# UBC-AWP/vision-sam3-yolo-lameless

Measured on AMD Instinct MI355X. Metric: frames/sec (whole node) for YOLO+SAM3+DINOv3 feature extraction, 1080p clips, higher is better.
Workload: dtype f16; 1 GPU; BASELINE cfg#5, dense schedule: fused per-frame path on a synthetic 5 s @ 30 fps 1080p clip (150 unique BGR frames resident in HBM): YOLOv8-l detect (letterbox 384x640, NMS, scale_boxes; f16 plan) -> SAM (Hiera-B+ image encoder + FPN at 1024x1024, box-prompted mask decoder, 1080p mask + statistics + contour features) + DINOv3 ViT-L/16 embed (224x224) on EVERY frame; per-frame records packed, gathe; parallelism=one clip per GPU, 1 GPU(s), one gather per step, streams=7

## Files before the change

### include/lmx.h

```cpp
#ifndef LMX_H
#define LMX_H
#include <stdint.h>
#ifdef __cplusplus
extern "C" {
#endif

#define LMX_VERSION 100

#define LMX_OK 0
#define LMX_EINVAL (-1)
#define LMX_EHIP (-2)

typedef void* lmx_stream_t;

int lmx_version(void);
const char* lmx_last_error(void);
int lmx_device_count(void);

enum { LMX_F16 = 0, LMX_F32 = 1 };
enum { LMX_ACT_NONE = 0, LMX_ACT_SILU = 1, LMX_ACT_GELU = 2 , LMX_ACT_RELU = 3,
       LMX_ACT_SWIGLU = 4  };

typedef struct {
  const void* A;
// ... 76 lines not shown
int lmx_k_nms(const float* pred, int n, int A, int nc, float conf, double iou, int max_det, float max_wh,
              float* boxes, float* scores, int32_t* cls, int32_t* src, int32_t* counts, void* workspace,
              lmx_stream_t stream);

int lmx_k_letterbox(const uint8_t* src, uint8_t* dst, int n, int sh, int sw, int rh, int rw, int top, int left,
                    int oh, int ow, const int32_t* xofs, const int16_t* ialpha, const int32_t* yofs,
                    const int16_t* ibeta, int swap_rb, lmx_stream_t stream);
int lmx_k_stem_conv(const uint8_t* img, const float* w, const float* bias, void* out, int n, int H, int W, int Cout,
                    lmx_stream_t stream);
int lmx_k_maxpool5(const void* src, int64_t lds, void* dst, int64_t ldd, int n, int H, int W, int C,
                   lmx_stream_t stream);
int lmx_k_upsample2(const void* src, int64_t lds, void* dst, int64_t ldd, int n, int H, int W, int C,
                    lmx_stream_t stream);
int lmx_k_detect_decode(const float* head, int64_t ldh, float* pred, int n, int H, int W, int nc, float stride,
                        int a_off, int A, lmx_stream_t stream);
int lmx_k_scale_boxes(float* boxes, int total, float padx, float pady, float gain, float w, float h,
                      lmx_stream_t stream);

int lmx_k_split3(const float* x, int64_t ldx, int act, const void* res3, int64_t ldr, void* out3, int64_t ldo, int64_t rows,
                 int N, int g, int nsum, int64_t sum_stride, lmx_stream_t stream);
int lmx_k_maxpool5_x3(const void* src3, int64_t lds, void* dst3, int64_t ldd, int n, int H, int W, int C, lmx_stream_t stream);
int lmx_k_stem_conv_x3(const uint8_t* img, const float* w, const float* bias, void* out3, int n, int H, int W, int Cout,
                       lmx_stream_t stream);
int lmx_k_attention_f32(const float* q, int64_t ldq, const float* k, int64_t ldk, const float* v, int64_t ldv, float* o,
                        int64_t ldo, int B, int H, int Tq, int Tk, int hd, float scale, lmx_stream_t stream);
int lmx_k_hyper_mask_f32(const float* up, const float* hyper, float* logits, int n, int G, int C, int act, lmx_stream_t stream);

int lmx_k_pose_gather(const float* raw0, const float* raw1, const float* raw2, int64_t ldk, const int32_t* hw,
                      const float* strides, const int32_t* src, const int32_t* counts, int n, int max_det, int K, int ndim,
                      float padx, float pady, float gain, float w, float h, float* out, lmx_stream_t stream);

int lmx_k_im2col_u8(const uint8_t* img, const float* lut, void* out, int n, int rh, int rw, int IH, int IW, int KH,
                    int KW, int stride, int pad, int64_t ldo, lmx_stream_t stream);
int lmx_k_maxpool2(const void* src, int64_t lds, void* dst, int64_t ldd, int dtype, int n, int H, int W, int C,
                   lmx_stream_t stream);
int lmx_k_cast_f32_f16(const float* src, int64_t lds, void* dst, int64_t ldd, int64_t rows, int cols,
                       lmx_stream_t stream);

int lmx_k_add_bcast(const void* a, int a_dtype, int64_t lda, const float* b, int64_t ldb, int b_rows, void* out,
                    int out_dtype, int64_t ldo, int64_t rows, int D, lmx_stream_t stream);
int lmx_k_prompt_box(const float* boxes, int64_t ldb, float* sparse, int n, double sx, double sy, float S,
                     const float* gauss, const float* corner, int F, lmx_stream_t stream);
int lmx_k_hyper_mask(const void* up, const float* hyper, float* logits, int n, int G, int C, lmx_stream_t stream);
int lmx_k_mask_post(const float* logits, int n, int L, int T, int nh, int nw, int h, int w, uint8_t* mask,
                    int64_t* stats, float* workspace, lmx_stream_t stream);
int lmx_k_prompt_points(const float* points, const int32_t* labels, int Np, const float* boxes, int64_t ldb, float* sparse, int n,
                        double sx, double sy, float S, const float* gauss, const float* point_embed, const float* not_a_point,
                        const float* corner, int F, lmx_stream_t stream);
#define LMX_MASK_EMBED_PARAMS 4684
int lmx_k_mask_embed(const float* mask_input, const void* emb, int emb_dtype, int64_t lde, const float* params, float* keys,
                     int64_t ldk, int n, int G, lmx_stream_t stream);
int lmx_k_hyper_mask_multi(const void* up, const float* hyper, float* logits, int n, int M, int G, int C, lmx_stream_t stream);
int lmx_k_hyper_mask_multi_f32(const float* up, const float* hyper, float* logits, int n, int M, int G, int C, int act,
                               lmx_stream_t stream);
int lmx_k_mask_logits(const float* logits, int n, int L, int T, int nh, int nw, int h, int w, float* out, lmx_stream_t stream);

int lmx_k_mask_score(const float* logits, int n, int L, int T, int nh, int nw, int h, int w, double thr, double off,
                     const int32_t* idx, int64_t* out, lmx_stream_t stream);
int lmx_k_nms_boxes(const float* boxes, int64_t ldb, const float* scores, const uint8_t* valid, int n, double iou, int32_t* keep_out,
                    int32_t* count_out, void* workspace, lmx_stream_t stream);
int lmx_k_pack_bits(const uint8_t* src, int64_t rows, int w, uint8_t* dst, lmx_stream_t stream);

int64_t lmx_contour_workspace_bytes(int n, int h, int w);
int lmx_k_contour_features(const uint8_t* mask, int n, int h, int w, int64_t* out, void* workspace, lmx_stream_t stream);

int lmx_h_mask_features(const uint8_t* mask_host, int h, int w, double* out_host);
// ... 9 lines not shown
```

### vision-sam3-yolo-lameless_amd/csrc/nms.hip

```cpp
#include "common.h"

namespace {

constexpr int MAX_A = 16384;

__global__ __launch_bounds__(256) void nms_filter_kernel(const float* __restrict__ pred, int n, int A, int nc,
                                                         float conf, unsigned long long* __restrict__ keys,
                                                         int* __restrict__ counts) {
  const int64_t total = (int64_t)n * A;
  const int row_len = 4 + nc;
  for (int64_t i = (int64_t)blockIdx.x * blockDim.x + threadIdx.x; i < total; i += (int64_t)gridDim.x * blockDim.x) {
    const int img = (int)(i / A);
    const int a = (int)(i - (int64_t)img * A);
    const float* row = pred + i * row_len + 4;
    float best = row[0];
    for (int c = 1; c < nc; ++c) {
      const float v = row[c];
      best = v > best ? v : best;
    }
    if (best > conf) {
      const int slot = atomicAdd(&counts[img], 1);
      const unsigned long long key =
          ((unsigned long long)__float_as_uint(best) << 32) | (unsigned long long)(0xFFFFFFFFu - (unsigned)a);
      keys[(int64_t)img * A + slot] = key;
    }
  }
}

struct Box {
  float x1, y1, x2, y2, area;
};

__device__ __forceinline__ bool iou_gt(const Box& a, const Box& b, double thr) {
  const float xx1 = a.x1 > b.x1 ? a.x1 : b.x1;
  const float yy1 = a.y1 > b.y1 ? a.y1 : b.y1;
  const float xx2 = a.x2 < b.x2 ? a.x2 : b.x2;
  const float yy2 = a.y2 < b.y2 ? a.y2 : b.y2;
  float w = xx2 - xx1;
  w = w > 0.f ? w : 0.f;
  float h = yy2 - yy1;
  h = h > 0.f ? h : 0.f;
  const float inter = w * h;
  const float ovr = inter / (a.area + b.area - inter);
  return (double)ovr > thr;
}

__device__ __forceinline__ void bitonic_sort_desc(unsigned long long* keys, int npow2) {
  const int tid = threadIdx.x;
  for (int k = 2; k <= npow2; k <<= 1) {
    for (int j = k >> 1; j > 0; j >>= 1) {
      for (int i = tid; i < npow2; i += 1024) {
        const int ixj = i ^ j;
        if (ixj > i) {
          const unsigned long long a = keys[i], b = keys[ixj];
          const bool desc = (i & k) == 0;
          if (desc ? (a < b) : (a > b)) {
            keys[i] = b;
// ... 199 lines not shown
    sbox[i * 5 + 2] = r[2];
    sbox[i * 5 + 3] = r[3];
    sbox[i * 5 + 4] = (r[2] - r[0]) * (r[3] - r[1]);
  }
  __syncthreads();

  const int total = greedy_blocks(sbox, count, iou, count, supp, kept, [&](int, int i, int o) {
    keep_out[o] = (int)(0xFFFFFFFFu - (unsigned)(keys[i] & 0xFFFFFFFFull));
  });
  if (tid == 0) count_out[0] = total;
}

}

extern "C" int64_t lmx_nms_workspace_bytes(int n, int A) {
  if (n <= 0 || A <= 0) return 0;
  return 256 + ((int64_t)n * 4 + 255) / 256 * 256 + (int64_t)n * A * 8 + (int64_t)n * A * 5 * 4;
}

extern "C" int lmx_k_nms(const float* pred, int n, int A, int nc, float conf, double iou, int max_det, float max_wh,
                         float* boxes, float* scores, int32_t* cls, int32_t* src, int32_t* counts, void* workspace,
                         lmx_stream_t stream) {
  LMX_REQUIRE(pred && boxes && scores && cls && src && counts && workspace, "lmx_k_nms: null pointer");
  LMX_REQUIRE(n > 0 && A > 0 && A <= MAX_A && nc > 0 && max_det > 0, "lmx_k_nms: n=%d A=%d (<=%d) nc=%d max_det=%d", n,
              A, MAX_A, nc, max_det);
  LMX_REQUIRE((((uintptr_t)workspace) & 255) == 0, "lmx_k_nms: workspace must be 256-byte aligned");
  hipStream_t st = reinterpret_cast<hipStream_t>(stream);
  char* ws = reinterpret_cast<char*>(workspace);
  int* cand_counts = reinterpret_cast<int*>(ws);
  const int64_t cnt_bytes = ((int64_t)n * 4 + 255) / 256 * 256;
  unsigned long long* keys = reinterpret_cast<unsigned long long*>(ws + cnt_bytes);
  float* sbox = reinterpret_cast<float*>(ws + cnt_bytes + (int64_t)n * A * 8);
  LMX_HIP(hipMemsetAsync(cand_counts, 0, (size_t)n * 4, st));
  int64_t g = ((int64_t)n * A + 255) / 256;
  if (g > 2048) g = 2048;
  hipLaunchKernelGGL(nms_filter_kernel, dim3((unsigned)g), dim3(256), 0, st, pred, n, A, nc, conf, keys, cand_counts);
  int rc = lmx_launch_check("nms_filter_kernel");
  if (rc) return rc;
  int npow2 = 64;
  while (npow2 < A) npow2 <<= 1;
  const size_t smem = (size_t)npow2 * 9 + 64 * sizeof(Box);
  int dev;
  LMX_TRY(lmx_stream_device(st, &dev));
  LMX_TRY(lmx_allow_lds(reinterpret_cast<const void*>(&nms_greedy_kernel), (int)((size_t)MAX_A * 9 + 64 * sizeof(Box)), dev));
  hipLaunchKernelGGL(nms_greedy_kernel, dim3(n), dim3(1024), smem, st, pred, A, nc, iou, max_det, max_wh, keys, cand_counts,
                     sbox, boxes, scores, cls, src, counts);
  return lmx_launch_check("nms_greedy_kernel");
}

extern "C" int lmx_k_nms_boxes(const float* boxes, int64_t ldb, const float* scores, const uint8_t* valid, int n, double iou,
                               int32_t* keep_out, int32_t* count_out, void* workspace, lmx_stream_t stream) {
  LMX_REQUIRE(boxes && scores && keep_out && count_out && workspace, "lmx_k_nms_boxes: null pointer");
  LMX_REQUIRE(n > 0 && n <= MAX_A && ldb >= 4, "lmx_k_nms_boxes: n=%d (1..%d) ldb=%lld", n, MAX_A, (long long)ldb);
  LMX_REQUIRE((((uintptr_t)workspace) & 15) == 0, "lmx_k_nms_boxes: workspace must be 16-byte aligned");
  int npow2 = 64;
  while (npow2 < n) npow2 <<= 1;
  const size_t smem = (size_t)npow2 * 9 + 64 * sizeof(Box);
  hipStream_t st = reinterpret_cast<hipStream_t>(stream);
  int dev;
  LMX_TRY(lmx_stream_device(st, &dev));
  LMX_TRY(lmx_allow_lds(reinterpret_cast<const void*>(&nms_boxes_kernel), (int)((size_t)MAX_A * 9 + 64 * sizeof(Box)), dev));
  hipLaunchKernelGGL(nms_boxes_kernel, dim3(1), dim3(1024), smem, st, boxes, ldb, scores, valid, n, iou, reinterpret_cast<float*>(workspace),
                     keep_out, count_out);
  return lmx_launch_check("nms_boxes_kernel");
}
```

### vision-sam3-yolo-lameless_amd/csrc/sam.hip

```cpp
#include "common.h"

namespace {

inline int grid_for(int64_t total, int block = 256) {
  int64_t g = (total + block - 1) / block;
  if (g > 256 * 8) g = 256 * 8;
  if (g < 1) g = 1;
  return (int)g;
}

template <int KW_T>
__global__ __launch_bounds__(256) void im2col_u8_kernel(const uint8_t* __restrict__ img, const float* __restrict__ lut,
                                                        half_t* __restrict__ out, int n, int rh, int rw, int OH, int OW, int KH,
                                                        int KW_rt, int stride, int pad, int64_t ldo) {
  __shared__ float lut_s[768];
  for (int i = threadIdx.x; i < 768; i += blockDim.x) lut_s[i] = lut[i];
  __syncthreads();
  const int KW = KW_T > 0 ? KW_T : KW_rt;
  const int chunks = (int)(ldo / 8);
  const int K = KH * KW * 3;
  const int64_t total = (int64_t)n * OH * OW * chunks;
  for (int64_t i = (int64_t)blockIdx.x * blockDim.x + threadIdx.x; i < total; i += (int64_t)gridDim.x * blockDim.x) {
    const int ck = (int)(i % chunks);
    const int64_t tok = i / chunks;
// ... 253 lines not shown
    if (fast) {
      x = *reinterpret_cast<const unsigned long long*>(sp);
    } else {
      for (int e = 0; e < 8; ++e)
        if (c * 8 + e < w) x |= (unsigned long long)sp[e] << (8 * e);
    }
    x = (x | (x >> 1) | (x >> 2) | (x >> 3) | (x >> 4) | (x >> 5) | (x >> 6) | (x >> 7)) & 0x0101010101010101ull;
    dst[i] = (uint8_t)((x * 0x8040201008040201ull) >> 56);
  }
}

__global__ __launch_bounds__(256) void prompt_box_kernel(const float* __restrict__ boxes, int64_t ldb, float* __restrict__ sparse,
                                                        int n, double sx, double sy, float S, const float* __restrict__ gauss,
                                                        const float* __restrict__ corner, int F) {
  const int i = blockIdx.x * blockDim.x + threadIdx.x;
  if (i >= n * 2 * F) return;
  const int j = i % F, k = (i / F) & 1, b = i / (2 * F);
  const float* bx = boxes + (int64_t)b * ldb + 2 * k;
  const float px = (float)((double)bx[0] * sx) + 0.5f, py = (float)((double)bx[1] * sy) + 0.5f;
  const float cx = 2.f * (px / S) - 1.f, cy = 2.f * (py / S) - 1.f;
  const float ang = 6.283185307179586f * (cx * gauss[j] + cy * gauss[F + j]);
  float* o = sparse + ((int64_t)b * 2 + k) * 2 * F;
  o[j] = sinf(ang) + corner[k * 2 * F + j];
  o[F + j] = cosf(ang) + corner[k * 2 * F + F + j];
}

__global__ void mask_stats_init_kernel(long long* stats, int n) {
  const int i = blockIdx.x * blockDim.x + threadIdx.x;
  if (i >= n * 8) return;
  const int f = i & 7;
  stats[i] = (f == 3 || f == 4) ? 0x7fffffffll : ((f == 5 || f == 6) ? -1ll : 0ll);
}

}

extern "C" int lmx_k_im2col_u8(const uint8_t* img, const float* lut, void* out, int n, int rh, int rw, int IH, int IW, int KH,
                               int KW, int stride, int pad, int64_t ldo, lmx_stream_t stream) {
  LMX_REQUIRE(img && lut && out, "lmx_k_im2col_u8: null pointer");
  LMX_REQUIRE(n > 0 && rh > 0 && rw > 0 && rh <= IH && rw <= IW && KH > 0 && KW > 0 && stride > 0 && pad >= 0,
              "lmx_k_im2col_u8: geometry");
  LMX_REQUIRE(ldo % 8 == 0 && ldo >= (int64_t)KH * KW * 3 && aligned16(out), "lmx_k_im2col_u8: ldo/alignment");
  const int OH = (IH + 2 * pad - KH) / stride + 1, OW = (IW + 2 * pad - KW) / stride + 1;
  LMX_REQUIRE((int64_t)rh * rw * 3 < 0x7fffffffll, "lmx_k_im2col_u8: frame too large");
  const dim3 grid(grid_for((int64_t)n * OH * OW * (ldo / 8)));
  hipStream_t st = reinterpret_cast<hipStream_t>(stream);
  half_t* o16 = reinterpret_cast<half_t*>(out);
  if (KW == 7)
    hipLaunchKernelGGL((im2col_u8_kernel<7>), grid, dim3(256), 0, st, img, lut, o16, n, rh, rw, OH, OW, KH, KW, stride, pad, ldo);
  else if (KW == 16)
    hipLaunchKernelGGL((im2col_u8_kernel<16>), grid, dim3(256), 0, st, img, lut, o16, n, rh, rw, OH, OW, KH, KW, stride, pad, ldo);
  else
    hipLaunchKernelGGL((im2col_u8_kernel<0>), grid, dim3(256), 0, st, img, lut, o16, n, rh, rw, OH, OW, KH, KW, stride, pad, ldo);
  return lmx_launch_check("im2col_u8_kernel");
}

extern "C" int lmx_k_maxpool2(const void* src, int64_t lds, void* dst, int64_t ldd, int dtype, int n, int H, int W, int C,
                              lmx_stream_t stream) {
  LMX_REQUIRE(src && dst, "lmx_k_maxpool2: null pointer");
  LMX_REQUIRE(n > 0 && H > 0 && W > 0 && H % 2 == 0 && W % 2 == 0 && C > 0 && lds >= C && ldd >= C, "lmx_k_maxpool2: shape");
  hipStream_t st = reinterpret_cast<hipStream_t>(stream);
  if (dtype == LMX_F16) {
    LMX_REQUIRE(C % 8 == 0 && lds % 8 == 0 && ldd % 8 == 0 && aligned16(src) && aligned16(dst), "lmx_k_maxpool2: f16 alignment");
    hipLaunchKernelGGL((maxpool2_kernel<half_t, 8>), dim3(grid_for((int64_t)n * (H / 2) * (W / 2) * (C / 8))), dim3(256), 0, st,
                       reinterpret_cast<const half_t*>(src), lds, reinterpret_cast<half_t*>(dst), ldd, n, H, W, C);
  } else if (dtype == LMX_F32) {
    LMX_REQUIRE(C % 4 == 0 && lds % 4 == 0 && ldd % 4 == 0 && aligned16(src) && aligned16(dst), "lmx_k_maxpool2: f32 alignment");
    hipLaunchKernelGGL((maxpool2_kernel<float, 4>), dim3(grid_for((int64_t)n * (H / 2) * (W / 2) * (C / 4))), dim3(256), 0, st,
                       reinterpret_cast<const float*>(src), lds, reinterpret_cast<float*>(dst), ldd, n, H, W, C);
  } else {
    LMX_REQUIRE(false, "lmx_k_maxpool2: dtype %d", dtype);
  }
  return lmx_launch_check("maxpool2_kernel");
}

extern "C" int lmx_k_cast_f32_f16(const float* src, int64_t lds, void* dst, int64_t ldd, int64_t rows, int cols,
                                  lmx_stream_t stream) {
  LMX_REQUIRE(src && dst, "lmx_k_cast_f32_f16: null pointer");
  LMX_REQUIRE(rows > 0 && cols > 0 && cols % 4 == 0 && lds % 4 == 0 && ldd % 4 == 0 && lds >= cols && ldd >= cols,
              "lmx_k_cast_f32_f16: shape");
  LMX_REQUIRE(aligned16(src) && ((((uintptr_t)dst) & 7) == 0), "lmx_k_cast_f32_f16: alignment");
  hipLaunchKernelGGL(cast_kernel, dim3(grid_for(rows * (cols / 4))), dim3(256), 0, reinterpret_cast<hipStream_t>(stream), src, lds,
                     reinterpret_cast<half_t*>(dst), ldd, rows, cols);
  return lmx_launch_check("cast_kernel");
}

extern "C" int lmx_k_prompt_box(const float* boxes, int64_t ldb, float* sparse, int n, double sx, double sy, float S,
// ... 81 lines not shown
```

### vision-sam3-yolo-lameless_amd/lmx/_lib.py

```python
import ctypes as C
import os

_HERE = os.path.dirname(os.path.abspath(__file__))
LIB_PATH = os.environ.get("LMX_LIB") or os.path.join(_HERE, "liblmx.so")


class LmxError(RuntimeError):
    pass


class GemmDesc(C.Structure):
    _fields_ = [
        ("A", C.c_void_p), ("W", C.c_void_p), ("bias", C.c_void_p), ("scale", C.c_void_p), ("res", C.c_void_p),
        ("C", C.c_void_p),
        ("lda", C.c_int64), ("ldc", C.c_int64), ("ldr", C.c_int64),
        ("M", C.c_int32), ("N", C.c_int32), ("K", C.c_int32),
        ("act", C.c_int32), ("out_dtype", C.c_int32), ("a_mode", C.c_int32),
        ("H", C.c_int32), ("W_", C.c_int32), ("Cin", C.c_int32), ("conv_stride", C.c_int32),
        ("Ho", C.c_int32), ("Wo", C.c_int32), ("res_rows", C.c_int32), ("a_rep", C.c_int32), ("split_k", C.c_int32), ("split_stride", C.c_int64),
    ]


class AttnDesc(C.Structure):
    _fields_ = [
# ... 16 lines not shown
    "lmx_dbg_set_gemm2_variant": (None, [_I]),
    "lmx_k_pose_gather": (_I, [_VP, _VP, _VP, _I64, _VP, _VP, _VP, _VP, _I, _I, _I, _I, _F, _F, _F, _F, _F, _VP, _VP]),
    "lmx_k_pack_bits": (_I, [_VP, _I64, _I, _VP, _VP]),
    "lmx_k_ln_mlp": (_I, [_VP, _I64, _VP, _VP, _VP, _VP, _VP, _VP, _I64, _I, _F, _VP, _VP, _VP, _VP, _VP, _VP]),
    "lmx_k_hiera_attn8": (_I, [_VP, _VP, _I64, _VP, _VP, _F, _VP, _VP, _VP, _VP, _I, _I, _I, _I, _I, _F, _VP]),
    "lmx_k_hiera_attn4": (_I, [_VP, _VP, _I64, _VP, _VP, _I, _I, _I, _I, _I, _F, _VP]),
    "lmx_k_hiera_attn_pool": (_I, [_VP, _VP, _VP, _VP, _I, _I, _I, _I, _I, _I, _F, _VP]),
    "lmx_k_ln_mlp_img": (_I, [_VP, _I64, _VP, _VP, _I64, _I, _F, _VP, _VP, _VP]),
    "lmx_k_layernorm": (_I, [_VP, _I, _I64, _VP, _VP, _VP, _I, _I64, _I, _I, _F, _I, _VP]),
    "lmx_k_attention": (_I, [C.POINTER(AttnDesc), _VP]),
    "lmx_k_relpos_tables": (_I, [C.POINTER(AttnDesc), _VP, _VP, _I, _VP, _VP]),
    "lmx_k_rope": (_I, [_VP, _I64, _I, _I, _I, _I, _I, _VP, _VP, _VP]),
    "lmx_k_pil_resize_h": (_I, [_VP, _VP, _I, _I, _I, _I, _VP, _VP, _I, _I, _VP]),
    "lmx_k_pil_resize_v": (_I, [_VP, _VP, _I, _I, _I, _I, _VP, _VP, _I, _VP]),
    "lmx_k_patchify_norm": (_I, [_VP, _VP, _I, _I, _I, _I, _I, _I, _I, _I, _I64, _VP, _VP]),
    "lmx_k_float_resize_patchify": (_I, [_VP, _VP, _I, _I, _I, _I, _I, _I, _I64, _VP, _VP, _I, _VP, _VP, _I, _I, _F, _VP, _I, _VP]),
    "lmx_k_assemble_tokens": (_I, [_VP, _VP, _VP, _VP, _I, _I, _I, _I, _VP]),
    "lmx_k_token_mean": (_I, [_VP, _I, _VP, _I, _I, _I, _VP]),
    "lmx_k_swiglu": (_I, [_VP, _I64, _VP, _I64, _I, _I, _VP]),
    "lmx_nms_workspace_bytes": (_I64, [_I, _I]),
    "lmx_k_nms": (_I, [_VP, _I, _I, _I, _F, _D, _I, _F, _VP, _VP, _VP, _VP, _VP, _VP, _VP]),
    "lmx_k_letterbox": (_I, [_VP, _VP, _I, _I, _I, _I, _I, _I, _I, _I, _I, _VP, _VP, _VP, _VP, _I, _VP]),
    "lmx_k_stem_conv": (_I, [_VP, _VP, _VP, _VP, _I, _I, _I, _I, _VP]),
    "lmx_k_split3": (_I, [_VP, _I64, _I, _VP, _I64, _VP, _I64, _I64, _I, _I, _I, _I64, _VP]),
    "lmx_k_maxpool5_x3": (_I, [_VP, _I64, _VP, _I64, _I, _I, _I, _I, _VP]),
    "lmx_k_stem_conv_x3": (_I, [_VP, _VP, _VP, _VP, _I, _I, _I, _I, _VP]),
    "lmx_k_attention_f32": (_I, [_VP, _I64, _VP, _I64, _VP, _I64, _VP, _I64, _I, _I, _I, _I, _I, _F, _VP]),
    "lmx_k_hyper_mask_f32": (_I, [_VP, _VP, _VP, _I, _I, _I, _I, _VP]),
    "lmx_k_maxpool5": (_I, [_VP, _I64, _VP, _I64, _I, _I, _I, _I, _VP]),
    "lmx_k_upsample2": (_I, [_VP, _I64, _VP, _I64, _I, _I, _I, _I, _VP]),
    "lmx_k_detect_decode": (_I, [_VP, _I64, _VP, _I, _I, _I, _I, _F, _I, _I, _VP]),
    "lmx_k_scale_boxes": (_I, [_VP, _I, _F, _F, _F, _F, _F, _VP]),
    "lmx_k_im2col_u8": (_I, [_VP, _VP, _VP, _I, _I, _I, _I, _I, _I, _I, _I, _I, _I64, _VP]),
    "lmx_k_maxpool2": (_I, [_VP, _I64, _VP, _I64, _I, _I, _I, _I, _I, _VP]),
    "lmx_k_cast_f32_f16": (_I, [_VP, _I64, _VP, _I64, _I64, _I, _VP]),
    "lmx_k_add_bcast": (_I, [_VP, _I, _I64, _VP, _I64, _I, _VP, _I, _I64, _I64, _I, _VP]),
    "lmx_h_mask_features": (_I, [_VP, _I, _I, _VP]),
    "lmx_h_iou_matrix": (_I, [_VP, _I, _VP, _I, _VP]),
    "lmx_h_assign": (_I, [_VP, _I, _I, _VP, _VP]),
    "lmx_contour_workspace_bytes": (_I64, [_I, _I, _I]),
    "lmx_k_contour_features": (_I, [_VP, _I, _I, _I, _VP, _VP, _VP]),
    "lmx_k_prompt_box": (_I, [_VP, _I64, _VP, _I, _D, _D, _F, _VP, _VP, _I, _VP]),
    "lmx_k_hyper_mask": (_I, [_VP, _VP, _VP, _I, _I, _I, _VP]),
    "lmx_k_mask_post": (_I, [_VP, _I, _I, _I, _I, _I, _I, _I, _VP, _VP, _VP, _VP]),
    "lmx_k_prompt_points": (_I, [_VP, _VP, _I, _VP, _I64, _VP, _I, _D, _D, _F, _VP, _VP, _VP, _VP, _I, _VP]),
    "lmx_k_mask_embed": (_I, [_VP, _VP, _I, _I64, _VP, _VP, _I64, _I, _I, _VP]),
    "lmx_k_hyper_mask_multi": (_I, [_VP, _VP, _VP, _I, _I, _I, _I, _VP]),
    "lmx_k_hyper_mask_multi_f32": (_I, [_VP, _VP, _VP, _I, _I, _I, _I, _I, _VP]),
    "lmx_k_mask_logits": (_I, [_VP, _I, _I, _I, _I, _I, _I, _I, _VP, _VP]),
    "lmx_k_mask_score": (_I, [_VP, _I, _I, _I, _I, _I, _I, _I, _D, _D, _VP, _VP, _VP]),
    "lmx_k_nms_boxes": (_I, [_VP, _I64, _VP, _VP, _I, _D, _VP, _VP, _VP, _VP]),
}

_lib = None


def load():
    global _lib
    if _lib is not None:
        return _lib
    if not os.path.exists(LIB_PATH):
        raise ImportError(
            f"{LIB_PATH} not found: build it with `python -c 'import __graft_entry__ as g; g.build()'` "
            "(hipcc --offload-arch=gfx950).  lmx has no CPU fallback.")
    import torch

# ... 14 lines not shown
```

### vision-sam3-yolo-lameless_amd/lmx/kernels.py

```python
import ctypes as C
import os
import threading

import torch

from . import _lib
from ._lib import AttnDesc, GemmDesc, LmxError, check

F16, F32 = 0, 1
ACT_NONE, ACT_SILU, ACT_GELU, ACT_RELU, ACT_SWIGLU = 0, 1, 2, 3, 4
_DT = {torch.float16: F16, torch.float32: F32}


_tls = threading.local()


def _stream(dev):
    _tls.dev = dev
    return C.c_void_p(torch.cuda.current_stream(dev).cuda_stream)


def _ptr(t):
    return C.c_void_p(t.data_ptr()) if t is not None else C.c_void_p(0)

# ... 42 lines not shown
        raise LmxError(f"gemm: out shape {tuple(out.shape)} != ({Mout},{Nout})")
    d = GemmDesc()
    d.A, d.W, d.C = a.data_ptr(), w.data_ptr(), out.data_ptr()
    d.bias = bias.data_ptr() if bias is not None else None
    d.scale = scale.data_ptr() if scale is not None else None
    d.lda, d.ldc, d.ldr = lda, ldc, 0
    if bias is not None and (bias.dtype != torch.float32 or bias.numel() != N):
        raise LmxError("gemm: bias must be float32 [N]")
    if scale is not None and (scale.dtype != torch.float32 or scale.numel() != Nout):
        raise LmxError("gemm: scale must be float32 [N] (ACT_SWIGLU: [N/2])")
    if res is not None:
        Mr, Nr, ldr = _rows(res, "gemm res")
        if (Mr, Nr) != ((res_rows or M), N) or res.dtype != out.dtype:
            raise LmxError("gemm: residual must match out's shape and dtype")
        d.res, d.ldr = res.data_ptr(), ldr
    d.res_rows = res_rows
    d.M, d.N, d.K = M, N, a_rep * K
    d.act, d.out_dtype, d.a_mode, d.a_rep = act, _DT[out.dtype], 0, a_rep
    if pool_hw:
        d.a_mode, d.H, d.W_ = 2, int(pool_hw[0]), int(pool_hw[1])
    check(_lib.load().lmx_k_gemm(C.byref(d), _stream(dev)), "lmx_k_gemm")
    return out


def im2col_u8(img, lut, IH, IW, KH, KW, stride, pad, ldo):
    dev = _dev(img, lut)
    n, rh, rw, c = img.shape
    if c != 3 or img.dtype != torch.uint8 or not img.is_contiguous():
        raise LmxError("im2col_u8: img must be contiguous uint8 [n,h,w,3]")
    OH, OW = (IH + 2 * pad - KH) // stride + 1, (IW + 2 * pad - KW) // stride + 1
    out = torch.empty((n * OH * OW, ldo), dtype=torch.float16, device=img.device)
    check(_lib.load().lmx_k_im2col_u8(_ptr(img), _ptr(lut), _ptr(out), n, rh, rw, IH, IW, KH, KW, stride, pad, ldo,
                                      _stream(dev)), "lmx_k_im2col_u8")
    return out


def maxpool2(x, out):
    dev = _dev(x, out)
    n, H, W, Cc, ps = _nhwc(x, "maxpool2 x")
    no, Ho, Wo, Co, pso = _nhwc(out, "maxpool2 out")
    if (no, Ho, Wo, Co) != (n, H // 2, W // 2, Cc) or x.dtype != out.dtype:
        raise LmxError("maxpool2: shape/dtype mismatch")
    check(_lib.load().lmx_k_maxpool2(_ptr(x), ps, _ptr(out), pso, _DT[x.dtype], n, H, W, Cc, _stream(dev)), "lmx_k_maxpool2")
    return out


def cast_f16(x, out=None):
    dev = _dev(x, out)
    rows, cols, lds = _rows(x, "cast src")
    if out is None:
        out = torch.empty((rows, cols), dtype=torch.float16, device=x.device)
    check(_lib.load().lmx_k_cast_f32_f16(_ptr(x), lds, _ptr(out), out.stride(0), rows, cols, _stream(dev)),
          "lmx_k_cast_f32_f16")
    return out


def _nhwc(t, what):
    if t.dim() != 4 or t.stride(3) != 1:
        raise LmxError(f"{what}: expected NHWC with contiguous channels, got {tuple(t.shape)} / {t.stride()}")
    n, H, W, Cc = t.shape
    ps = t.stride(2)
    if t.stride(1) != W * ps or (n > 1 and t.stride(0) != H * W * ps):
        raise LmxError(f"{what}: not a channel slice of a dense NHWC buffer: strides {t.stride()}")
    return n, H, W, Cc, ps


# ... 661 lines not shown
                                      _stream(dev)), "lmx_k_nms_boxes")
    return keep, count


def contour_features(mask):
    dev = _dev(mask)
    if mask.dtype != torch.uint8 or mask.dim() != 3 or not mask.is_contiguous():
        raise LmxError("contour_features: mask must be contiguous uint8 [n,h,w]")
    n, h, w = mask.shape
    lib = _lib.load()
    ws = torch.empty((int(lib.lmx_contour_workspace_bytes(n, h, w)),), dtype=torch.uint8, device=mask.device)
    out = torch.empty((n, 8), dtype=torch.int64, device=mask.device)
    check(lib.lmx_k_contour_features(_ptr(mask), n, h, w, _ptr(out), _ptr(ws), _stream(dev)), "lmx_k_contour_features")
    return out


LAUNCH_TRACE = None
_raw_lib = None
RIDGE_FLOP_PER_BYTE = 2500e12 / 8e12


def _work(name, args):
    if name == "lmx_k_gemm":
        d = args[0]._obj
        M, N, Kd = d.M, d.N, d.K
        osz = 4 if d.out_dtype == F32 else 2
        a_bytes = 2 * M * (Kd // max(d.a_rep, 1))
        if d.a_mode == 1:
            a_bytes = 2 * (M // max(d.Ho * d.Wo, 1)) * d.H * d.W_ * d.Cin
        by = a_bytes + 2 * N * Kd + osz * (M // 4 if d.a_mode == 2 else M) * (N // 2 if d.act == ACT_SWIGLU else N) + (osz * (d.res_rows or M) * N if d.res else 0)
        fl = 2.0 * M * N * Kd
        key = f"gemm M={M} N={N} K={Kd} out={'f32' if osz == 4 else 'f16'} conv3x3={d.a_mode} act={d.act} res={int(bool(d.res))}"
        return ("gemm/mfma-bound" if fl / by >= RIDGE_FLOP_PER_BYTE else "gemm/hbm-bound"), fl, by, key
    if name == "lmx_k_attention":
        d = args[0]._obj
        fl = 4.0 * d.B * d.H * d.Tq * d.Tk * d.hd
        by = 2 * d.H * d.hd * d.B * (2 * d.Tq + 2 * d.Tk)
        key = f"attention B={d.B} H={d.H} Tq={d.Tq} Tk={d.Tk} hd={d.hd} mode={d.mode} ws={d.ws} qs={d.q_stride} rel={int(bool(d.rel))}"
        return ("attention/mfma-bound" if fl / by >= RIDGE_FLOP_PER_BYTE else "attention/hbm-bound"), fl, by, key
    if name == "lmx_k_layernorm":
        in_dt, out_dt, rows, D = args[1], args[6], args[8], args[9]
        return "layernorm", 0.0, rows * D * ((4 if in_dt == F32 else 2) + (4 if out_dt == F32 else 2)), f"layernorm rows={rows} D={D} in={in_dt} out={out_dt}"
    if name == "lmx_k_ln_mlp_img":
        rows, D = args[4], args[5]
        return "fused ln+mlp", 16.0 * D * D * rows, (8 + (2 if args[7] else 0) + (2 if args[8] else 0)) * D * rows, f"ln_mlp_img rows={rows} D={D}"
    if name == "lmx_k_ln_mlp":
        rows, D = args[8], args[9]
        return "fused ln+mlp", 16.0 * D * D * rows, (16 + (2 if args[12] else 0) + (2 if args[15] else 0)) * D * rows, f"ln_mlp rows={rows} D={D}"
    if name == "lmx_k_hiera_attn8":
        n_, Gh, Gw, D = args[10], args[11], args[12], args[13]
        rows = n_ * Gh * Gw
        return "fused attention half", rows * (8.0 * D * D + 256.0 * D), rows * D * (8 + (2 if args[0] else 0)), f"hiera_attn8 rows={rows} D={D} ln_inside={int(not args[0])}"
    if name == "lmx_k_hiera_attn4":
        n_, Gh, Gw, D = args[5], args[6], args[7], args[8]
        rows = n_ * Gh * Gw
        return "fused attention half", rows * (8.0 * D * D + 64.0 * D), rows * D * 10, f"hiera_attn4 rows={rows} D={D}"
    if name == "lmx_k_hiera_attn_pool":
        n_, Gh, Gw, Di, Do = args[4], args[5], args[6], args[7], args[8]
        rows = n_ * Gh * Gw
        keys = 64 if Di == 112 else 16
        return "fused attention half", rows * (8.0 * Di * Do + keys * Do + 0.5 * Do * Do), rows * (2 * Di + Do), f"hiera_attn_pool rows={rows} {Di}->{Do}"
    if name == "lmx_k_cast_f32_f16":
        rows, cols = args[4], args[5]
        return "streaming glue", 0.0, 6 * rows * cols, f"cast_f32_f16 rows={rows} cols={cols}"
    if name == "lmx_k_maxpool2":
        dt, n_, H, W, C_ = args[4], args[5], args[6], args[7], args[8]
# ... 67 lines not shown
```

### vision-sam3-yolo-lameless_amd/lmx/sam.py

```python
import math
import os
from dataclasses import dataclass

import numpy as np
import torch

from . import kernels as K
from . import resample

SAM_PIXEL_MEAN = (123.675, 116.28, 103.53)
SAM_PIXEL_STD = (58.395, 57.12, 57.375)


@dataclass
class HieraConfig:
    hidden: int = 112
    blocks: tuple = (2, 3, 16, 3)
    dims: tuple = (112, 224, 448, 896)
    heads: tuple = (2, 4, 8, 16)
    windows: tuple = (8, 4, 14, 7)
    global_blocks: tuple = (12, 16, 20)
    pos_bkg: tuple = (14, 14)
    q_pool_stages: int = 3
    fpn_dim: int = 256
# ... 267 lines not shown
                nx = f"backbone.blocks.{i + 1}." if i + 1 < len(self.blocks) else None
                f32 = lambda k: np.asarray(sd[k], np.float32)
                blk["mlp_img"] = tuple(torch.from_numpy(a).to(dev) for a in pack_ln_mlp(
                    f32(p + "mlp.proj_in.weight"), f32(p + "mlp.proj_in.bias"), f32(p + "mlp.proj_out.weight"), f32(p + "mlp.proj_out.bias"),
                    f32(p + "layer_norm2.weight"), f32(p + "layer_norm2.bias"),
                    f32(nx + "layer_norm1.weight") if nx else None, f32(nx + "layer_norm1.bias") if nx else None))
        n = len(cfg.dims) - 1
        self.neck = [(t16(sd[f"neck.convs.{n - i}.weight"][:, :, 0, 0]), t32(sd[f"neck.convs.{n - i}.bias"])) for i in range(n + 1)]
        self.lut = t32(sam_norm_lut())
        self._tabs = {}

    def _tables(self, h, w):
        key = (h, w)
        if key not in self._tabs:
            nh, nw = resize_longest_side(h, w, self.cfg.image)
            dev = self.device

            def up(tab):
                b, k, ks = tab
                return (torch.from_numpy(b).to(dev), torch.from_numpy(k).to(dev), ks)

            th = up(resample.coeff_tables(w, nw, resample.BILINEAR)) if nw != w else None
            tv = up(resample.coeff_tables(h, nh, resample.BILINEAR)) if nh != h else None
            self._tabs[key] = (nh, nw, th, tv)
        return self._tabs[key]

    def preprocess(self, frames):
        n, h, w, _ = frames.shape
        nh, nw, th, tv = self._tables(h, w)
        img = K.pil_resize(frames, nw, nh, th, tv, swap_rb=False)
        S = self.cfg.image
        return img, K.im2col_u8(img, self.lut, S, S, 7, 7, 4, 3, self.k_pad)

    def trunk(self, patches, n):
        cfg = self.cfg
        g = self.grid0
        x = K.gemm(patches, self.pe_w, bias=self.pe_b, res=self.pos, res_rows=g * g, out_dtype=torch.float32)
        H = W = g
        stage_ends = set(int(v) for v in np.cumsum(cfg.blocks) - 1)
        stages, stages16 = [], []
        dev = x.device
        h_next = None
        for i, B in enumerate(self.blocks):
            dim, D, heads, qs = B["dim"], B["dim_out"], B["heads"], B["qs"]
            rows = n * H * W
            if self._attn8(i, H, W):
                if B["attn8_ln"]:
                    K.hiera_attn8(x, B["attn8"], n, H, W, heads, ln=(B["g1"], B["b1"], cfg.eps))
                else:
                    K.hiera_attn8(x, B["attn8"], n, H, W, heads, h=h_next if h_next is not None else K.layernorm(x, B["g1"], B["b1"], cfg.eps))
            elif "attnp" in B and K.hiera_attn_pool_ok(dim, D, heads, B["win"], H, W, qs):
                x = K.hiera_attn_pool(h_next if h_next is not None else K.layernorm(x, B["g1"], B["b1"], cfg.eps), B["attnp"], n, H, W, heads, D)
                H, W = H // 2, W // 2
            elif "attn4" in B and K.hiera_attn4_ok(D, heads, B["win"], H, W, qs):
                K.hiera_attn4(h_next if h_next is not None else K.layernorm(x, B["g1"], B["b1"], cfg.eps), x, B["attn4"], n, H, W, heads)
            else:
                h = h_next if h_next is not None else K.layernorm(x, B["g1"], B["b1"], cfg.eps)
                if dim != D:
                    if qs and K.pooled_gemm_ok(rows, D):
                        sc = K.gemm(h, B["wp"], bias=B["bp"], out_dtype=torch.float32, pool_hw=(H, W))
                    else:
                        sc = K.gemm(h, B["wp"], bias=B["bp"], out_dtype=torch.float32)
                        if qs:
                            pooled = torch.empty((n, H // 2, W // 2, D), dtype=torch.float32, device=dev)
                            K.maxpool2(sc.view(n, H, W, D), pooled)
                            sc = pooled.view(-1, D)
                    res = sc
                else:
                    res = x
                x, H, W = self._attention_half(B, h, x, res, n, H, W)
# ... 52 lines not shown
                        window=dict(Gh=H, Gw=W, ws=win, q_stride=2 if qs else 1),
                        pad_k=B["padkv"][D:2 * D], pad_v=B["padkv"][2 * D:])
        else:
            K.attention(q, k, v, a, n, heads, Hq * Wq, H * W, hd, hd ** -0.5)
        xo = torch.empty((n * Hq * Wq, D), dtype=torch.float32, device=dev) if res is not x else x
        K.gemm(a, B["wo"], bias=B["bo"], res=res, out=xo)
        return xo, Hq, Wq

    def fpn(self, stages, stages16=None):
        cfg = self.cfg
        nlev = len(stages) - 1
        feats, prev = [], None
        for i in range(nlev, -1, -1):
            s = stages[i]
            n, H, W, C = s.shape
            a = stages16[i] if stages16 and stages16[i] is not None else K.cast_f16(s.view(-1, C))
            w, b = self.neck[i]
            out = torch.empty((n, H, W, cfg.fpn_dim), dtype=torch.float16, device=s.device)
            if i not in cfg.fpn_top_down or i == nlev:
                K.gemm(a, w, bias=b, out=out.view(-1, cfg.fpn_dim))
            else:
                up = torch.empty((n, H, W, cfg.fpn_dim), dtype=torch.float16, device=s.device)
                K.upsample2(prev, up)
                K.gemm(a, w, bias=b, res=up.view(-1, cfg.fpn_dim), out=out.view(-1, cfg.fpn_dim))
            prev = out
            feats.append(out)
        return feats[-3:][::-1]

    def encode_patches(self, patches, n):
        stages, stages16 = self.trunk(patches, n)
        return dict(fpn=self.fpn(stages, stages16), stages=stages)

    def encode(self, frames, precision=None):
        img, patches = self.preprocess(frames)
        out = self.encode_patches(patches, frames.shape[0])
        out["resized"] = img
        return out


@dataclass
class SamVitConfig:
    hidden: int = 768
    layers: int = 12
    heads: int = 12
    mlp: int = 3072
    global_idx: tuple = (2, 5, 8, 11)
    window: int = 14
    patch: int = 16
    image: int = 1024
    out_ch: int = 256
    eps: float = 1e-6

    @property
    def grid(self):
        return self.image // self.patch


def sam_vit_b():
    return SamVitConfig()


def sam_vit_l():
    return SamVitConfig(hidden=1024, layers=24, heads=16, mlp=4096, global_idx=(5, 11, 17, 23))


def sam_vit_h():
    return SamVitConfig(hidden=1280, layers=32, heads=16, mlp=5120, global_idx=(7, 15, 23, 31))

# ... 151 lines not shown
```

Baseline: 684.5 frames/s.

## Fuse Hiera patch-embed im2col and GEMM into one kernel; wave-parallel NMS filter

Adds a patch-embed kernel for the Hiera 7x7/stride-4 stem. It stages a LUT-normalised uint8 image tile in LDS and runs MFMA with weights held in registers, adding bias and the positional residual in the same pass. This removes the materialised f16 im2col buffer and the separate GEMM launch. The NMS candidate filter is also rewritten so lanes in a wave cooperate on each anchor's class max (optionally vectorised) and slots are allocated with one ballot-based atomic per wave instead of per-thread atomics. Risks are a hand-rolled kernel valid only for one conv geometry and N<=112, and a different candidate order, since slot assignment changes.

```diff
diff --git a/include/lmx.h b/include/lmx.h
--- a/include/lmx.h
+++ b/include/lmx.h
@@ -132,6 +132,9 @@
 
 int lmx_k_im2col_u8(const uint8_t* img, const float* lut, void* out, int n, int rh, int rw, int IH, int IW, int KH,
                     int KW, int stride, int pad, int64_t ldo, lmx_stream_t stream);
+int lmx_k_patch_embed_u8(const uint8_t* img, const float* lut, int n, int rh, int rw, int IH, int IW, int KH, int KW,
+                         int stride, int pad, const void* w, int64_t ldw, const float* bias, const float* res, int64_t ldr,
+                         int res_rows, float* out, int64_t ldc, int N, lmx_stream_t stream);
 int lmx_k_maxpool2(const void* src, int64_t lds, void* dst, int64_t ldd, int dtype, int n, int H, int W, int C,
                    lmx_stream_t stream);
 int lmx_k_cast_f32_f16(const float* src, int64_t lds, void* dst, int64_t ldd, int64_t rows, int cols,
diff --git a/vision-sam3-yolo-lameless_amd/csrc/nms.hip b/vision-sam3-yolo-lameless_amd/csrc/nms.hip
--- a/vision-sam3-yolo-lameless_amd/csrc/nms.hip
+++ b/vision-sam3-yolo-lameless_amd/csrc/nms.hip
@@ -4,25 +4,67 @@
 
 constexpr int MAX_A = 16384;
 
-__global__ __launch_bounds__(256) void nms_filter_kernel(const float* __restrict__ pred, int n, int A, int nc,
+template <int VEC>
+__global__ __launch_bounds__(256) void nms_filter_kernel(const float* __restrict__ pred, int n, int A, int nc, int lg,
                                                          float conf, unsigned long long* __restrict__ keys,
                                                          int* __restrict__ counts) {
-  const int64_t total = (int64_t)n * A;
+  const int lane = threadIdx.x & 63;
+  const int G = 1 << lg, apw = 64 >> lg;
+  const int g = lane & (G - 1), grp = lane >> lg;
   const int row_len = 4 + nc;
-  for (int64_t i = (int64_t)blockIdx.x * blockDim.x + threadIdx.x; i < total; i += (int64_t)gridDim.x * blockDim.x) {
-    const int img = (int)(i / A);
-    const int a = (int)(i - (int64_t)img * A);
-    const float* row = pred + i * row_len + 4;
-    float best = row[0];
-    for (int c = 1; c < nc; ++c) {
-      const float v = row[c];
-      best = v > best ? v : best;
-    }
-    if (best > conf) {
-      const int slot = atomicAdd(&counts[img], 1);
-      const unsigned long long key =
-          ((unsigned long long)__float_as_uint(best) << 32) | (unsigned long long)(0xFFFFFFFFu - (unsigned)a);
-      keys[(int64_t)img * A + slot] = key;
+  const int units = nc / VEC;
+  const int cpi = (A + 63) / 64;
+  const int64_t nchunk = (int64_t)n * cpi;
+  for (int64_t ch = (int64_t)blockIdx.x * 4 + (threadIdx.x >> 6); ch < nchunk; ch += (int64_t)gridDim.x * 4) {
+    const int img = (int)(ch / cpi);
+    const int a0 = (int)(ch - (int64_t)img * cpi) * 64;
+    float mine = 0.f;
+    for (int it = 0; it < G; ++it) {
+      const int a = a0 + it * apw + grp;
+      float best = -__builtin_inff();
+      int bi = 0x7fffffff;
+      if (a < A) {
+        const float* cls = pred + ((int64_t)img * A + a) * row_len + 4;
+        for (int u = g; u < units; u += G) {
+          if (VEC == 4) {
+            const f32x4 v = *reinterpret_cast<const f32x4*>(cls + u * 4);
+#pragma unroll
+            for (int e = 0; e < 4; ++e)
+              if (v[e] > best) {
+                best = v[e];
+                bi = u * 4 + e;
+              }
+          } else {
+            const float v = cls[u];
+            if (v > best) {
+              best = v;
+              bi = u;
+            }
+          }
+        }
+      }
+      for (int o = G >> 1; o > 0; o >>= 1) {
+        const float ob = __shfl_xor(best, o, 64);
+        const int oi = __shfl_xor(bi, o, 64);
+        if (ob > best || (ob == best && oi < bi)) {
+          best = ob;
+          bi = oi;
+        }
+      }
+      const float r = __shfl(best, (lane & (apw - 1)) << lg, 64);
+      if ((lane >> (6 - lg)) == it) mine = r;
+    }
+    const int a = a0 + lane;
+    const bool pass = a < A && mine > conf;
+    const unsigned long long m = __ballot(pass);
+    if (m == 0ull) continue;
+    int base = 0;
+    if (lane == 0) base = atomicAdd(&counts[img], __popcll(m));
+    base = __shfl(base, 0, 64);
+    if (pass) {
+      const int slot = base + __popcll(m & ((1ull << lane) - 1ull));
+      keys[(int64_t)img * A + slot] =
+          ((unsigned long long)__float_as_uint(mine) << 32) | (unsigned long long)(0xFFFFFFFFu - (unsigned)a);
     }
   }
 }
@@ -288,9 +330,16 @@
   unsigned long long* keys = reinterpret_cast<unsigned long long*>(ws + cnt_bytes);
   float* sbox = reinterpret_cast<float*>(ws + cnt_bytes + (int64_t)n * A * 8);
   LMX_HIP(hipMemsetAsync(cand_counts, 0, (size_t)n * 4, st));
-  int64_t g = ((int64_t)n * A + 255) / 256;
-  if (g > 2048) g = 2048;
-  hipLaunchKernelGGL(nms_filter_kernel, dim3((unsigned)g), dim3(256), 0, st, pred, n, A, nc, conf, keys, cand_counts);
+  const bool vec4 = nc % 4 == 0 && aligned16(pred);
+  const int units = vec4 ? nc / 4 : nc;
+  int lg = 0;
+  while (lg < 4 && (1 << lg) < units) ++lg;
+  int64_t g = ((int64_t)n * ((A + 63) / 64) + 3) / 4;
+  if (g > 8192) g = 8192;
+  if (vec4)
+    hipLaunchKernelGGL(nms_filter_kernel<4>, dim3((unsigned)g), dim3(256), 0, st, pred, n, A, nc, lg, conf, keys, cand_counts);
+  else
+    hipLaunchKernelGGL(nms_filter_kernel<1>, dim3((unsigned)g), dim3(256), 0, st, pred, n, A, nc, lg, conf, keys, cand_counts);
   int rc = lmx_launch_check("nms_filter_kernel");
   if (rc) return rc;
   int npow2 = 64;
diff --git a/vision-sam3-yolo-lameless_amd/csrc/sam.hip b/vision-sam3-yolo-lameless_amd/csrc/sam.hip
--- a/vision-sam3-yolo-lameless_amd/csrc/sam.hip
+++ b/vision-sam3-yolo-lameless_amd/csrc/sam.hip
@@ -309,6 +309,133 @@
   stats[i] = (f == 3 || f == 4) ? 0x7fffffffll : ((f == 5 || f == 6) ? -1ll : 0ll);
 }
 
+
+namespace pe {
+constexpr int T = 16;
+constexpr int RP = T * 4 + 3;
+constexpr int ROWH = RP * 3;
+constexpr int NF = 7, NKS = 5;
+constexpr int KREAL = 147;
+constexpr int ERS = NF * 16 + 4;
+constexpr int S_HALFS = (RP * ROWH + 7) / 8 * 8;
+constexpr int DW = (ROWH + 3 + 3) / 4;
+constexpr int NLD = (RP * DW + 511) / 512 * 2;
+}
+
+__global__ __launch_bounds__(256, 2) void patch_embed_u8_kernel(const uint8_t* __restrict__ img, const float* __restrict__ lut,
+                                                                const half_t* __restrict__ W, int ldw, const float* __restrict__ bias,
+                                                                const float* __restrict__ res, int64_t ldr, int res_rows,
+                                                                float* __restrict__ C, int64_t ldc, int rh, int rw, int OH, int OW,
+                                                                int N, int tiles_x, int tiles_y, int ntiles) {
+  using namespace pe;
+  __shared__ __attribute__((aligned(16))) half_t S[S_HALFS];
+  __shared__ __attribute__((aligned(16))) float E[4 * T * ERS];
+  __shared__ __attribute__((aligned(16))) float bias_s[NF * 16];
+  __shared__ half_t lut_h[768];
+  const int tid = threadIdx.x, lane = tid & 63;
+  const int wave = __builtin_amdgcn_readfirstlane(tid >> 6);
+  const int frow = lane & 15, fq = lane >> 4;
+  for (int i = tid; i < 768; i += 256) lut_h[i] = (half_t)lut[i];
+  if (tid < NF * 16) bias_s[tid] = (tid < N && bias) ? bias[tid] : 0.f;
+
+  half8_t wf[NKS][NF];
+#pragma unroll
+  for (int kt = 0; kt < NKS; ++kt)
+#pragma unroll
+    for (int j = 0; j < NF; ++j) {
+      const int nrow = j * 16 + frow, k = kt * 32 + fq * 8;
+      wf[kt][j] = half8_t{0, 0, 0, 0, 0, 0, 0, 0};
+      if (nrow < N && k < ldw) wf[kt][j] = *reinterpret_cast<const half8_t*>(W + (int64_t)nrow * ldw + k);
+    }
+
+  float* Ew = E + wave * (T * ERS);
+  const int nq = N >> 2;
+  for (int tile = blockIdx.x; tile < ntiles; tile += gridDim.x) {
+    const int b = tile / (tiles_x * tiles_y), rem = tile - b * (tiles_x * tiles_y);
+    const int ty = rem / tiles_x, tx = rem - ty * tiles_x;
+    const int oy0 = ty * T, ox0 = tx * T;
+    const int yb = oy0 * 4 - 3, xb = ox0 * 4 - 3;
+    const uint8_t* ib = img + (int64_t)b * rh * rw * 3;
+    __syncthreads();
+    const uintptr_t ibp = reinterpret_cast<uintptr_t>(ib);
+    const int jlo = xb < 0 ? -xb * 3 : 0;
+    const int jhi = (rw - xb) * 3 < ROWH ? (rw - xb) * 3 : ROWH;
+    for (int h = 0; h < 2; ++h) {
+    unsigned rg[NLD / 2];
+#pragma unroll
+    for (int i = 0; i < NLD / 2; ++i) {
+      const int t = tid + (h * (NLD / 2) + i) * 256, sy = t / DW, d = t - sy * DW, y = yb + sy;
+      const uintptr_t a0 = ibp + ((int64_t)y * rw + xb) * 3;
+      const int j0 = 4 * d - (int)(a0 & 3);
+      rg[i] = 0u;
+      if (t < RP * DW && (unsigned)y < (unsigned)rh && j0 + 3 >= jlo && j0 < jhi)
+        rg[i] = *reinterpret_cast<const unsigned*>((a0 & ~(uintptr_t)3) + 4 * d);
+    }
+#pragma unroll
+    for (int i = 0; i < NLD / 2; ++i) {
+      const int t = tid + (h * (NLD / 2) + i) * 256, sy = t / DW, d = t - sy * DW, y = yb + sy;
+      const uintptr_t a0 = ibp + ((int64_t)y * rw + xb) * 3;
+      const int j0 = 4 * d - (int)(a0 & 3);
+      const bool row_ok = (unsigned)y < (unsigned)rh;
+      if (t < RP * DW) {
+#pragma unroll
+        for (int e = 0; e < 4; ++e) {
+          const int j = j0 + e;
+          if ((unsigned)j < (unsigned)ROWH) {
+            const int c = j % 3;
+            const half_t v = lut_h[c * 256 + ((rg[i] >> (8 * e)) & 255u)];
+            S[sy * ROWH + j] = (row_ok && j >= jlo && j < jhi) ? v : (half_t)0.f;
+          }
+        }
+      }
+    }
+    }
+    __syncthreads();
+    for (int rb = 0; rb < 4; ++rb) {
+      const int oyl = wave * 4 + rb, oy = oy0 + oyl;
+      if (oy >= OH) break;
+      f32x4 acc[NF];
+#pragma unroll
+      for (int j = 0; j < NF; ++j) acc[j] = f32x4{0.f, 0.f, 0.f, 0.f};
+      const half_t* Sb = S + oyl * 4 * ROWH + frow * 12;
+#pragma unroll
+      for (int kt = 0; kt < NKS; ++kt) {
+        half8_t af;
+#pragma unroll
+        for (int e = 0; e < 8; ++e) {
+          const int k = kt * 32 + fq * 8 + e;
+          const int ky = k / 21, kj = k - ky * 21;
+          const bool real = kt < NKS - 1 || k < KREAL;
+          const half_t v = Sb[real ? ky * ROWH + kj : 0];
+          af[e] = real ? v : (half_t)0.f;
+        }
+#pragma unroll
+        for (int j = 0; j < NF; ++j) acc[j] = __builtin_amdgcn_mfma_f32_16x16x32_f16(wf[kt][j], af, acc[j], 0, 0, 0);
+      }
+#pragma unroll
+      for (int j = 0; j < NF; ++j)
+        if (j * 16 < N)
+          *reinterpret_cast<f32x4*>(Ew + frow * ERS + j * 16 + fq * 4) = acc[j] + *reinterpret_cast<const f32x4*>(bias_s + j * 16 + fq * 4);
+      const int m_row0 = (b * OH + oy) * OW + ox0;
+      const int mr0 = res_rows > 0 ? m_row0 % res_rows : m_row0;
+      const int c4 = (lane & 31) * 4;
+#pragma unroll 2
+      for (int i = 0; i < T / 2; ++i) {
+        const int row = 2 * i + (lane >> 5);
+        if ((lane & 31) < nq && ox0 + row < OW) {
+          f32x4 o = *reinterpret_cast<const f32x4*>(Ew + row * ERS + c4);
+          if (res) {
+            int mr = mr0 + row;
+            if (res_rows > 0 && mr >= res_rows) mr %= res_rows;
+            o += *reinterpret_cast<const f32x4*>(res + (int64_t)mr * ldr + c4);
+          }
+          *reinterpret_cast<f32x4*>(C + (int64_t)(m_row0 + row) * ldc + c4) = o;
+        }
+      }
+    }
+  }
+}
+
 }
 
 extern "C" int lmx_k_im2col_u8(const uint8_t* img, const float* lut, void* out, int n, int rh, int rw, int IH, int IW, int KH,
@@ -329,6 +456,33 @@
   else
     hipLaunchKernelGGL((im2col_u8_kernel<0>), grid, dim3(256), 0, st, img, lut, o16, n, rh, rw, OH, OW, KH, KW, stride, pad, ldo);
   return lmx_launch_check("im2col_u8_kernel");
+}
+
+extern "C" int lmx_k_patch_embed_u8(const uint8_t* img, const float* lut, int n, int rh, int rw, int IH, int IW, int KH, int KW,
+                                    int stride, int pad, const void* w, int64_t ldw, const float* bias, const float* res, int64_t ldr,
+                                    int res_rows, float* out, int64_t ldc, int N, lmx_stream_t stream) {
+  LMX_REQUIRE(img && lut && w && bias && out, "lmx_k_patch_embed_u8: null pointer");
+  LMX_REQUIRE(n > 0 && rh > 0 && rw > 0 && rh <= IH && rw <= IW, "lmx_k_patch_embed_u8: geometry");
+  LMX_REQUIRE(KH == 7 && KW == 7 && stride == 4 && pad == 3,
+              "lmx_k_patch_embed_u8: built for Hiera's 7 x 7 / stride 4 / pad 3 patch convolution (got %d x %d / %d / %d): use "
+              "lmx_k_im2col_u8 + lmx_k_gemm", KH, KW, stride, pad);
+  LMX_REQUIRE(N > 0 && N % 16 == 0 && N <= pe::NF * 16, "lmx_k_patch_embed_u8: N=%d must be a multiple of 16, at most %d", N, pe::NF * 16);
+  LMX_REQUIRE(ldw % 8 == 0 && ldw >= pe::KREAL && ldw <= pe::NKS * 32 && aligned16(w), "lmx_k_patch_embed_u8: weight rows of ldw=%lld halfs (147..160, a multiple of 8), 16-byte aligned", (long long)ldw);
+  LMX_REQUIRE(ldc % 4 == 0 && ldc >= N && aligned16(out) && aligned16(bias), "lmx_k_patch_embed_u8: out / bias alignment, ldc=%lld", (long long)ldc);
+  LMX_REQUIRE(res_rows >= 0 && (!res || (ldr % 4 == 0 && ldr >= N && aligned16(res))), "lmx_k_patch_embed_u8: residual ldr=%lld res_rows=%d", (long long)ldr, res_rows);
+  const int OH = (IH + 2 * pad - KH) / stride + 1, OW = (IW + 2 * pad - KW) / stride + 1;
+  LMX_REQUIRE((int64_t)rh * rw * 3 < 0x7fffffffll && (int64_t)n * OH * OW < 0x7fffffffll, "lmx_k_patch_embed_u8: problem too large");
+  const int tiles_x = (OW + pe::T - 1) / pe::T, tiles_y = (OH + pe::T - 1) / pe::T;
+  const int64_t ntiles = (int64_t)n * tiles_x * tiles_y;
+  hipStream_t st = reinterpret_cast<hipStream_t>(stream);
+  int dev;
+  LMX_TRY(lmx_stream_device(st, &dev));
+  const int cus = lmx_cu_count(dev);
+  if (cus < 0) return cus;
+  const int64_t grid = ntiles < 2ll * cus ? ntiles : 2ll * cus;
+  hipLaunchKernelGGL(patch_embed_u8_kernel, dim3((unsigned)grid), dim3(256), 0, st, img, lut, reinterpret_cast<const half_t*>(w), (int)ldw,
+                     bias, res, ldr, res_rows, out, ldc, rh, rw, OH, OW, N, tiles_x, tiles_y, (int)ntiles);
+  return lmx_launch_check("patch_embed_u8_kernel");
 }
 
 extern "C" int lmx_k_maxpool2(const void* src, int64_t lds, void* dst, int64_t ldd, int dtype, int n, int H, int W, int C,
diff --git a/vision-sam3-yolo-lameless_amd/lmx/_lib.py b/vision-sam3-yolo-lameless_amd/lmx/_lib.py
--- a/vision-sam3-yolo-lameless_amd/lmx/_lib.py
+++ b/vision-sam3-yolo-lameless_amd/lmx/_lib.py
@@ -72,6 +72,7 @@
     "lmx_k_detect_decode": (_I, [_VP, _I64, _VP, _I, _I, _I, _I, _F, _I, _I, _VP]),
     "lmx_k_scale_boxes": (_I, [_VP, _I, _F, _F, _F, _F, _F, _VP]),
     "lmx_k_im2col_u8": (_I, [_VP, _VP, _VP, _I, _I, _I, _I, _I, _I, _I, _I, _I, _I64, _VP]),
+    "lmx_k_patch_embed_u8": (_I, [_VP, _VP, _I, _I, _I, _I, _I, _I, _I, _I, _I, _VP, _I64, _VP, _VP, _I64, _I, _VP, _I64, _I, _VP]),
     "lmx_k_maxpool2": (_I, [_VP, _I64, _VP, _I64, _I, _I, _I, _I, _I, _VP]),
     "lmx_k_cast_f32_f16": (_I, [_VP, _I64, _VP, _I64, _I64, _I, _VP]),
     "lmx_k_add_bcast": (_I, [_VP, _I, _I64, _VP, _I64, _I, _VP, _I, _I64, _I64, _I, _VP]),
diff --git a/vision-sam3-yolo-lameless_amd/lmx/kernels.py b/vision-sam3-yolo-lameless_amd/lmx/kernels.py
--- a/vision-sam3-yolo-lameless_amd/lmx/kernels.py
+++ b/vision-sam3-yolo-lameless_amd/lmx/kernels.py
@@ -98,6 +98,40 @@
     out = torch.empty((n * OH * OW, ldo), dtype=torch.float16, device=img.device)
     check(_lib.load().lmx_k_im2col_u8(_ptr(img), _ptr(lut), _ptr(out), n, rh, rw, IH, IW, KH, KW, stride, pad, ldo,
                                       _stream(dev)), "lmx_k_im2col_u8")
+    return out
+
+
+PATCH_EMBED_MAX_N = 112
+
+
+def patch_embed_u8_ok(KH, KW, stride, pad, N, ldw):
+    return (KH, KW, stride, pad) == (7, 7, 4, 3) and N % 16 == 0 and 0 < N <= PATCH_EMBED_MAX_N and ldw % 8 == 0 and 147 <= ldw <= 160
+
+
+def patch_embed_u8(img, lut, IH, IW, KH, KW, stride, pad, w, bias, res=None, res_rows=0, out=None):
+    dev = _dev(img, lut, w, bias, res, out)
+    n, rh, rw, c = img.shape
+    if c != 3 or img.dtype != torch.uint8 or not img.is_contiguous():
+        raise LmxError("patch_embed_u8: img must be contiguous uint8 [n,h,w,3]")
+    N, K, ldw = _rows(w, "patch_embed_u8 W")
+    if w.dtype != torch.float16 or ldw != K:
+        raise LmxError("patch_embed_u8: W must be contiguous float16 [N, k_pad]")
+    if bias is None or bias.dtype != torch.float32 or bias.numel() != N:
+        raise LmxError("patch_embed_u8: bias must be float32 [N]")
+    OH, OW = (IH + 2 * pad - KH) // stride + 1, (IW + 2 * pad - KW) // stride + 1
+    M = n * OH * OW
+    if out is None:
+        out = torch.empty((M, N), dtype=torch.float32, device=img.device)
+    Mo, No, ldc = _rows(out, "patch_embed_u8 out")
+    if (Mo, No) != (M, N) or out.dtype != torch.float32:
+        raise LmxError(f"patch_embed_u8: out must be float32 ({M},{N}), got {tuple(out.shape)}")
+    ldr = 0
+    if res is not None:
+        Mr, Nr, ldr = _rows(res, "patch_embed_u8 res")
+        if (Mr, Nr) != ((res_rows or M), N) or res.dtype != torch.float32:
+            raise LmxError("patch_embed_u8: residual must be float32 [res_rows or M, N]")
+    check(_lib.load().lmx_k_patch_embed_u8(_ptr(img), _ptr(lut), n, rh, rw, IH, IW, KH, KW, stride, pad, _ptr(w), ldw, _ptr(bias),
+                                           _ptr(res), ldr, res_rows, _ptr(out), ldc, N, _stream(dev)), "lmx_k_patch_embed_u8")
     return out
 
 
@@ -825,6 +859,12 @@
         fl = 2.0 * M * N * Kd
         key = f"gemm M={M} N={N} K={Kd} out={'f32' if osz == 4 else 'f16'} conv3x3={d.a_mode} act={d.act} res={int(bool(d.res))}"
         return ("gemm/mfma-bound" if fl / by >= RIDGE_FLOP_PER_BYTE else "gemm/hbm-bound"), fl, by, key
+    if name == "lmx_k_patch_embed_u8":
+        n_, rh, rw, IH, IW, KH, KW, st_, pad, ldw, rr, N = args[2], args[3], args[4], args[5], args[6], args[7], args[8], args[9], args[10], args[12], args[16], args[19]
+        M = n_ * ((IH + 2 * pad - KH) // st_ + 1) * ((IW + 2 * pad - KW) // st_ + 1)
+        by = 3 * n_ * rh * rw + 2 * N * ldw + 4 * M * N + (4 * (rr or M) * N if args[14] else 0)
+        fl = 2.0 * M * N * ldw
+        return ("gemm/mfma-bound" if fl / by >= RIDGE_FLOP_PER_BYTE else "gemm/hbm-bound"), fl, by, f"patch_embed_u8 M={M} N={N} K={ldw}"
     if name == "lmx_k_attention":
         d = args[0]._obj
         fl = 4.0 * d.B * d.H * d.Tq * d.Tk * d.hd
diff --git a/vision-sam3-yolo-lameless_amd/lmx/sam.py b/vision-sam3-yolo-lameless_amd/lmx/sam.py
--- a/vision-sam3-yolo-lameless_amd/lmx/sam.py
+++ b/vision-sam3-yolo-lameless_amd/lmx/sam.py
@@ -323,10 +323,20 @@
         S = self.cfg.image
         return img, K.im2col_u8(img, self.lut, S, S, 7, 7, 4, 3, self.k_pad)
 
-    def trunk(self, patches, n):
+    def embed(self, frames):
+        S, g = self.cfg.image, self.grid0
+        if not K.patch_embed_u8_ok(7, 7, 4, 3, self.cfg.hidden, self.k_pad):
+            img, patches = self.preprocess(frames)
+            return img, K.gemm(patches, self.pe_w, bias=self.pe_b, res=self.pos, res_rows=g * g, out_dtype=torch.float32)
+        n, h, w, _ = frames.shape
+        nh, nw, th, tv = self._tables(h, w)
+        img = K.pil_resize(frames, nw, nh, th, tv, swap_rb=False)
+        return img, K.patch_embed_u8(img, self.lut, S, S, 7, 7, 4, 3, self.pe_w, self.pe_b, res=self.pos, res_rows=g * g)
+
+    def trunk(self, patches, n, tokens=None):
         cfg = self.cfg
         g = self.grid0
-        x = K.gemm(patches, self.pe_w, bias=self.pe_b, res=self.pos, res_rows=g * g, out_dtype=torch.float32)
+        x = tokens if tokens is not None else K.gemm(patches, self.pe_w, bias=self.pe_b, res=self.pos, res_rows=g * g, out_dtype=torch.float32)
         H = W = g
         stage_ends = set(int(v) for v in np.cumsum(cfg.blocks) - 1)
         stages, stages16 = [], []
@@ -445,8 +455,9 @@
         return dict(fpn=self.fpn(stages, stages16), stages=stages)
 
     def encode(self, frames, precision=None):
-        img, patches = self.preprocess(frames)
-        out = self.encode_patches(patches, frames.shape[0])
+        img, tokens = self.embed(frames)
+        stages, stages16 = self.trunk(None, frames.shape[0], tokens=tokens)
+        out = dict(fpn=self.fpn(stages, stages16), stages=stages)
         out["resized"] = img
         return out
 
```

After: 691.2 frames/s, median of 6. About the same (+1.0%).
